# marsermd/DeepestScatter

Measured on AMD Instinct MI355X. Metric: Msamples/s (rays x spp) at 512^3 vol, 1024^2 frame; HBM GB/s vs roofline, higher is better.
Workload: dtype f32

## Files before the change

### deepestscatter_amd/_lib.py

```python
from __future__ import annotations

import ctypes as C
import os
from pathlib import Path

PKG = Path(__file__).resolve().parent
LIB_PATH = PKG / os.path.basename(os.environ.get("CT_LIBRARY", "libcloudtrace.so"))

CT_ABI_VERSION = 1
CT_OK, CT_E_INVAL, CT_E_HIP, CT_E_NOMEM, CT_E_STATE, CT_E_NODEVICE, CT_E_RCCL = 0, -1, -2, -3, -4, -5, -6
CT_MODE_SUN_AND_SKY_ALL_SCATTER, CT_MODE_SUN_MULTIPLE_SCATTER, CT_MODE_SUN_SINGLE_SCATTER = 0, 1, 2
CT_EST_MARCH, CT_EST_DELTA = 0, 1
CT_BUF_MEAN, CT_BUF_M2, CT_BUF_FRAME, CT_BUF_SCREEN, CT_BUF_INSCATTER, CT_BUF_DENSITY = range(6)
CT_FLAG_NONE, CT_FLAG_SIMPLE_KERNEL, CT_FLAG_LIGHT_NORMALIZED, CT_FLAG_SPARSE_BRICKS, CT_FLAG_VMM_BRICKS = 0, 1, 2, 4, 8
CT_FLAG_TEX_FIXED8 = 16

EXPORTS = [
    "ct_create", "ct_destroy", "ct_last_error", "ct_set_stream", "ct_set_camera", "ct_render_subframe",
    "ct_accumulate", "ct_render_accumulate", "ct_render_accumulate_async", "ct_synchronize", "ct_copy_to_device_async", "ct_point_radiance_launch", "ct_generate_scatter_samples", "ct_collect_descriptors", "ct_reset", "ct_tonemap", "ct_tonemap_async", "ct_set_render_ahead", "ct_rendered_subframes", "ct_set_stop_when_converged", "ct_converged_at", "ct_is_converged", "ct_tonemap_buffer", "ct_is_converged_buffers", "ct_download", "ct_upload",
    "ct_buffer_bytes", "ct_copy_to_device", "ct_device_ptr", "ct_subframes", "ct_set_subframes", "ct_counters", "ct_kernel_time",
    "ct_debug_cdf_inversion", "ct_debug_math_selftest", "ct_debug_fetch_probe", "ct_debug_fetch_probe_ws", "ct_debug_track_lines", "ct_debug_touched_lines", "ct_debug_stats", "ct_debug_stats_ex", "ct_debug_suspended", "ct_debug_timeline", "ct_debug_invariants", "ct_debug_memory", "ct_debug_delta_grid", "ct_debug_march_meta", "ct_fetch_counters", "ct_calculate_camera_variables", "ct_quantize_volume", "ct_load_vdb", "ct_generate_mipmaps",
    "ct_tile_owner", "ct_make_procedural_cloud",
    "ct_group_create", "ct_group_destroy", "ct_group_last_error", "ct_group_size", "ct_group_handle", "ct_group_set_camera",
    "ct_group_render_accumulate", "ct_group_reset", "ct_group_merge", "ct_group_download", "ct_group_tonemap",
    "ct_group_is_converged", "ct_group_counters",
]


class CtScene(C.Structure):
    _fields_ = [
        ("abi_version", C.c_uint32),
        ("dims", C.c_uint32 * 3),
        ("density_host", C.c_void_p),
        ("cloud_size_m", C.c_float),
        ("mean_free_path_m", C.c_float),
        ("sample_step", C.c_float),
# ... 86 lines not shown
        "ct_copy_to_device": (i32, [vp, i32, vp, C.c_size_t]),
        "ct_copy_to_device_async": (i32, [vp, i32, vp, C.c_size_t]),
        "ct_debug_suspended": (i32, [vp, vp]),
        "ct_debug_timeline": (i32, [vp, vp, u32]),
        "ct_device_ptr": (i32, [vp, i32, C.POINTER(vp)]),
        "ct_subframes": (i32, [vp, C.POINTER(u32)]),
        "ct_set_subframes": (i32, [vp, u32]),
        "ct_counters": (i32, [vp, C.POINTER(CtCounters)]),
        "ct_kernel_time": (i32, [vp, C.POINTER(C.c_double), C.POINTER(C.c_double), C.POINTER(C.c_uint64)]),
        "ct_debug_cdf_inversion": (i32, [vp, u32, u32, vp]),
        "ct_debug_math_selftest": (i32, [vp, i32, vp]),
        "ct_debug_stats": (i32, [vp, vp]),
        "ct_debug_stats_ex": (i32, [vp, vp, C.c_uint32]),
        "ct_debug_invariants": (i32, [vp, vp]),
        "ct_debug_memory": (i32, [vp, vp]),
        "ct_debug_delta_grid": (i32, [vp, vp]),
        "ct_debug_march_meta": (i32, [vp, vp, vp, C.c_size_t]),
        "ct_fetch_counters": (i32, [vp, C.POINTER(CtFetchCounters)]),
        "ct_debug_fetch_probe": (i32, [i32, u32, u32, C.POINTER(C.c_uint64)]),
        "ct_debug_fetch_probe_ws": (i32, [i32, u32, C.c_uint64, u32, C.POINTER(C.c_uint64)]),
        "ct_debug_track_lines": (i32, [vp, i32]),
        "ct_debug_touched_lines": (i32, [vp, C.POINTER(C.c_uint64), i32]),
        "ct_calculate_camera_variables": (i32, [vp, vp, vp, f32, f32, vp, vp, vp]),
        "ct_quantize_volume": (i32, [vp, vp, vp]),
        "ct_load_vdb": (i32, [C.c_char_p, vp, vp, C.c_size_t, C.POINTER(C.c_size_t), C.c_char_p, C.c_size_t]),
        "ct_generate_mipmaps": (i32, [vp, vp, vp, C.c_size_t, C.POINTER(u32), C.POINTER(C.c_size_t), vp]),
        "ct_tile_owner": (u32, [u32, u32, u32]),
        "ct_group_create": (i32, [C.POINTER(CtScene), vp, u32, C.POINTER(vp)]),
        "ct_group_destroy": (i32, [vp]),
        "ct_group_last_error": (C.c_char_p, [vp]),
# ... 25 lines not shown
```

### deepestscatter_amd/cloudtrace.py

```python
from __future__ import annotations

import ctypes as C
from dataclasses import dataclass
from pathlib import Path

import numpy as np

from . import _lib
from ._lib import (CT_BUF_DENSITY, CT_BUF_FRAME, CT_BUF_INSCATTER, CT_BUF_M2, CT_BUF_MEAN, CT_BUF_SCREEN,
                   CtCounters, CtFetchCounters, CtScene, check)

MIE_FILE = Path(__file__).resolve().parent / "data" / "mie_raw.f32"

LIGHT_DIRECTIONS = {
    "Front": (-0.586, -0.766, -0.271),
    "Side": (-0.03, -0.25, 0.8),
    "Back": (0.586, -0.766, -0.271),
}


def load_mie_raw() -> tuple[np.ndarray, np.ndarray]:
    raw = np.fromfile(MIE_FILE, dtype="<f4")
    if raw.size != 8192:
        raise RuntimeError(f"{MIE_FILE} is corrupt")
# ... 338 lines not shown
        c = CtFetchCounters()
        check(self.L.ct_fetch_counters(self.h, C.byref(c)), self.h)
        return c.as_dict()

    def debug_invariants(self) -> dict:
        out = np.zeros(8, np.uint64)
        check(self.L.ct_debug_invariants(self.h, _p(out)), self.h)
        names = ["armed", "checks", "violations", "samples_without_alpha_1", "dealt", "resumed", "written", "suspended"]
        return {n: int(v) for n, v in zip(names, out)}

    def debug_memory(self) -> dict:
        out = np.zeros(8, np.uint64)
        check(self.L.ct_debug_memory(self.h, _p(out)), self.h)
        names = ["raw_texture", "density_bricks", "inscatter_bricks", "march_bricks_dense", "march_bricks_stored", "sparse",
                 "row_table", "coarse_clearance"]
        return {n: int(v) for n, v in zip(names, out)}

    def delta_grid(self) -> dict:
        out = np.zeros(8, np.uint32)
        check(self.L.ct_debug_delta_grid(self.h, _p(out)), self.h)
        return {"cell": int(out[0]), "stored": tuple(int(v) for v in out[1:4]), "origin": tuple(int(v) for v in out[4:7]),
                "nee": int(out[7] & 0xff), "interior": bool(out[7] & 0x100)}

    def march_meta(self) -> dict:
        geom = np.zeros(8, np.uint32)
        check(self.L.ct_debug_march_meta(self.h, _p(geom), C.c_void_p(), 0), self.h)
        d = {"radius": int(geom[0]), "bias_x": int(geom[1]), "bias": int(geom[2]),
             "bricks": tuple(int(v) for v in geom[3:6]), "sparse": bool(geom[6]), "meta": None}
        if not d["sparse"]:
            gx, gy, gz = d["bricks"]
# ... 8 lines not shown
        return float(a.value), float(b.value), int(n.value)

    def set_stream(self, hip_stream: int | None):
        check(self.L.ct_set_stream(self.h, C.c_void_p(hip_stream) if hip_stream else None), self.h)

    def debug_stats(self) -> dict:
        out = np.zeros(64, np.uint64)
        check(self.L.ct_debug_stats(self.h, _p(out)), self.h)
        names = ["regen_phases", "regen_lanes", "march_phases", "march_lanes", "scatter_phases", "scatter_lanes",
                 "fetched_steps", "fetched_zero_cells", "skipped_steps", "zero_cells_nonfree_brick",
                 "zero_cells_free_brick_d1", "skip_loop_wave_iterations", "nee_footprints_reused", "waves",
                 "stolen_jobs", "max_scheduler_visits_of_a_wave"]
        d = {n: int(v) for n, v in zip(names, out)}
        d["wave_end_hist_5ms"] = [int(v) for v in out[16:40]]
        d["wave_end_minus_drained_hist_0p5ms"] = [int(v) for v in out[40:64]]
        ex = np.zeros(73, np.uint64)
        check(self.L.ct_debug_stats_ex(self.h, _p(ex), 73), self.h)
        d["march_fetch_same_line_as_lanes_previous"] = int(ex[68])
        d["march_fetch_line_shared_with_a_lower_lane"] = int(ex[69])
        d["nee_lookups_skipped_shadow_zero"] = int(ex[72])
        d["raw"] = [int(v) for v in out]
        d["watchdog"] = int(out[63])
        return d

    def debug_suspended(self) -> int:
        n = C.c_uint64(0)
        check(self.L.ct_debug_suspended(self.h, C.byref(n)), self.h)
        return int(n.value)

    def debug_math_selftest(self, which: int) -> dict:
        out = np.zeros(3, np.uint64)
        check(self.L.ct_debug_math_selftest(self.h, which, _p(out)), self.h)
        return {"tested": int(out[0]), "mismatches": int(out[1]), "first_bad_bits": int(out[2])}

    def debug_cdf_inversion(self, first_u24: int, count: int) -> np.ndarray:
# ... 81 lines not shown
```

### deepestscatter_amd/csrc/ct_api.cpp

```cpp
#include <algorithm>
#include <array>
#include <atomic>
#include <chrono>
#include <climits>
#include <cmath>
#include <cstdarg>
#include <cstdio>
#include <cstdlib>
#include <cstring>
#include <new>
#include <string>
#include <utility>
#include <map>
#include <vector>

#include "../../include/cloudtrace.h"
#include "ct_internal.hpp"

using namespace ct;

struct Knob {
    bool is_set = false;
    std::string text;
    const char *get() const { return is_set ? text.c_str() : nullptr; }
    explicit operator bool() const { return is_set; }
};
#define CT_KNOBS(X) X(BURST_IDLE) X(BURST_MARCH_MIN) X(BURST_SCATTER) X(CHUNK_INTERLEAVE) X(CHUNK_MORTON) X(CONTINUATION) X(DEBUG_INVARIANTS) X(DELTA_INTERIOR) X(DELTA_NEE) X(EXCHANGE) X(HAND_ON_JOBS) X(HINT_PERIOD) X(JOB_MAX) X(JOB_WORK) X(MARCH_BURST) X(MAX_AGE) X(NEE_CACHE) X(NO_ADVANCE) X(POINT_BLOCKS_PER_CU) X(POINT_ORDER) X(REGEN_MIN) X(RENDER_AHEAD) X(SCATTER_MIN) X(SCATTER_RATIO) X(SCRATCH_GIB) X(SCRATCH_MIB) X(SERPENTINE) X(SHARED_DEPTH) X(SPARSE) X(STATS) X(TAIL_BURST) X(TILE_ORDER) X(TIMELINE) X(TRACE) X(TUNE_SUBFRAMES) X(XCD_QUEUES) X(XCD_QUEUES_UNTUNED) X(XCD_REGIONS) X(BLOCKS_PER_CU)
struct CtTuning {
#define X(name) Knob name;
    CT_KNOBS(X)
#undef X
    static CtTuning from_env()
    {
        CtTuning t;
#define X(name)                                  \
    if (const char *e = getenv("CT_" #name)) {   \
        t.name.is_set = true;                    \
        t.name.text = e;                         \
    }
        CT_KNOBS(X)
#undef X
        return t;
// ... 70 lines not shown
    uint64_t scratch_cap_bytes = 0;
    uint32_t layout_S = 0;
    uint32_t *left[2] = { nullptr, nullptr };
    size_t left_capacity = 0;
    uint32_t *d_cont_count = nullptr;
    unsigned long long *d_cont_total = nullptr;
    size_t cont_capacity = 0;
    hipEvent_t ev_flush0 = nullptr, ev_flush1 = nullptr;
    bool continuation = true;
    int max_age_override = 0;
    bool hand_on_jobs = true;
    bool serpentine = false;
    float4 *d_primary = nullptr;
    float4 *d_advance = nullptr;
    uint32_t *d_pixels = nullptr;
    uint8_t *d_hit = nullptr, *hit_host = nullptr;
    uint32_t *d_cost = nullptr;
    uint32_t *d_touched[2] = { nullptr, nullptr };
    size_t touched_lines[2] = { 0, 0 };
    unsigned long long *d_timeline = nullptr;
    uint2 *d_cost_plane = nullptr;
    size_t cost_plane_capacity = 0;
    uint32_t *d_job_group = nullptr, *d_job_sub = nullptr;
    uint32_t n_groups = 0, groups_capacity = 0;
    uint32_t n_jobs = 0, jobs_capacity = 0, jobs_S = 0;
    uint32_t *jobs_host_g = nullptr, *jobs_host_s = nullptr;
    size_t jobs_host_capacity = 0;
    bool jobs_brief = false;
    uint32_t chunk_groups = 0, n_chunks = 0;
    std::vector<std::array<uint32_t, kQueues + 2>> chunk_q_begin;
// ... 258 lines not shown
    if (h->stream) {
        hipStreamSynchronize(h->stream);
    }
#ifdef CT_EXPERIMENTS
    if (h->vmm.va) {
        hipMemUnmap(h->vmm.va, h->vmm.size);
        for (auto &hd : h->vmm.handles) {
            hipMemRelease(hd);
        }
        hipMemAddressFree(h->vmm.va, h->vmm.size);
        h->vmm.va = nullptr;
        h->d_mbricks = nullptr;
    }
#endif
    void *ptrs[] = { h->d_density, h->d_inscatter, h->d_dbricks, h->d_ibricks, h->d_mbricks, h->d_tbricks, h->d_touched[0], h->d_touched[1], h->d_mrows, h->d_mcoarse, h->d_pyramid, h->d_mie, h->d_chopped, h->d_cdf,
                     h->d_guide, h->d_dist, h->d_dist_tmp, h->d_majorant, h->d_maj_cells, h->d_maj_codes, h->d_frame, h->d_mean, h->d_m2, h->d_screen, h->d_frames_all, h->cont[0], h->cont[1], h->left[0], h->left[1], h->d_cont_count, h->d_cont_total, h->d_primary, h->d_advance, h->d_pixels, h->d_cost, h->d_group_rank, h->d_group_order, h->d_job_group, h->d_job_sub, h->d_queue,
                     h->d_counters, h->d_colsum, h->d_avg, h->d_freeze, h->d_hit, h->d_cost_plane, h->d_timeline, h->pt.tasks, h->pt.primary, h->pt.frames, h->pt.pixels, h->pt.jg, h->pt.js };
    for (void *p : ptrs) {
        if (p) {
            hipFree(p);
        }
    }
    for (auto &e : h->ev) {
        if (e) {
            hipEventDestroy(e);
        }
    }
    for (auto &sl : h->slots) {
        if (sl.queue) {
            hipFree(sl.queue);
        }
// ... 358 lines not shown
    }
    if (delta) {
        d.delta_nee = (uint32_t)knob_int(t.DELTA_NEE, 0, 2, big ? 2 : 1);
        h->job_work = 48.f;
    }
    h->queues_enabled = knob_flag(t.XCD_QUEUES, big);
    h->regions = (uint32_t)knob_int(t.XCD_REGIONS, 1, 65536, (int)h->regions);
    if (const char *e = t.SHARED_DEPTH.get()) {
        h->shared_depth = (float)atof(e);
    }
    h->job_max = (uint32_t)knob_int(t.JOB_MAX, 1, 4096, (int)h->job_max);
    if (const char *e = t.JOB_WORK.get()) {
        h->job_work = (float)std::max(1.0, atof(e));
    }
    h->no_advance = knob_flag(t.NO_ADVANCE, h->no_advance);
    h->point_order = knob_flag(t.POINT_ORDER, h->point_order);
    h->continuation = knob_flag(t.CONTINUATION, h->continuation) && !h->exchange;
    h->chunk_interleave = knob_flag(t.CHUNK_INTERLEAVE, h->chunk_interleave);
    if (const char *e = t.TILE_ORDER.get()) {
        h->tile_hilbert = strcmp(e, "hilbert") == 0;
    }
    h->chunk_morton = knob_flag(t.CHUNK_MORTON, h->chunk_morton);
    h->serpentine = knob_flag(t.SERPENTINE, h->serpentine);
    h->hand_on_jobs = knob_flag(t.HAND_ON_JOBS, h->hand_on_jobs);
    h->max_age_override = knob_int(t.MAX_AGE, 0, CtHandle_::kMaxRegions - 1, h->max_age_override);
    h->ahead = (uint32_t)knob_int(t.RENDER_AHEAD, 0, 65535, (int)h->ahead);
    return CT_OK;
}

static void scene_uniforms(const CtScene *s, DevScene &d)
// ... 479 lines not shown
    NEED(h);
    if (!eye || !U || !V || !W) {
        return fail(h, CT_E_INVAL, "camera vectors must not be NULL");
    }
    DevScene &d = h->dev;
    d.ex = eye[0]; d.ey = eye[1]; d.ez = eye[2];
    d.ux = U[0]; d.uy = U[1]; d.uz = U[2];
    d.vx = V[0]; d.vy = V[1]; d.vz = V[2];
    d.wx = W[0]; d.wy = W[1]; d.wz = W[2];
    h->camera_set = true;
    h->queue_dirty = true;
    discard_ahead(h);
    return CT_OK;
}

static int rebuild_queue(CtHandle h)
{
    TracePhase trace(h, "rebuild_queue");
    const uint32_t W = h->scene.width, H = h->scene.height;
    const size_t pixels = (size_t)W * H;
    HIPCHK(h, launch_primary_rays(h->dev, h->d_primary, h->stream));
    if (h->scene.estimator == CT_EST_DELTA) {
        HIPCHK(h, launch_primary_advance_delta(h->dev, h->d_primary, h->d_advance, h->stream));
    } else {
        HIPCHK(h, launch_primary_advance(h->dev, h->d_primary, h->d_advance, h->stream));
    }
    if (!h->d_hit) {
        HIPCHK(h, dmalloc(&h->d_hit, pixels));
        HIPCHK(h, hipHostMalloc((void **)&h->hit_host, pixels, hipHostMallocDefault));
    }
// ... 67 lines not shown
                c >>= 1;
            }
            return k;
        };
        std::stable_sort(h->group_order.begin(), h->group_order.end(), [&](uint32_t a, uint32_t b) {
            return log2_class(h->tile_deepest[h->group_tile[a]]) > log2_class(h->tile_deepest[h->group_tile[b]]);
        });
    }
    h->group_depth.assign(h->n_groups, 0.f);
    if (h->n_groups) {
        HIPCHK(h, hipMemcpyAsync(h->d_pixels, list.data(), list.size() * sizeof(uint32_t), hipMemcpyHostToDevice,
                                 h->stream));
        HIPCHK(h, hipMemsetAsync(h->d_cost, 0, 2 * (size_t)h->n_groups * sizeof(uint32_t), h->stream));
        HIPCHK(h, hipStreamSynchronize(h->stream));
    }
    h->queue_dirty = false;
    h->order_tuned = false;
    h->jobs_S = 0;
    return CT_OK;
}

static bool short_batch(CtHandle h, uint32_t S)
{
    return h->scene.estimator != CT_EST_DELTA && (double)S * (double)std::max<uint64_t>(h->hit_pixels, 1) < 4.0e7;
}

static int build_jobs(CtHandle h, uint32_t S, uint32_t chunk_groups)
{
    chunk_groups = std::max(1u, std::min(chunk_groups, std::max(h->n_groups, 1u)));
    if (h->jobs_S >= S && h->jobs_brief == short_batch(h, S) && h->chunk_groups == chunk_groups) {
// ... 439 lines not shown
        } else {
            HIPCHK(h, launch_render_delta_x(sc, ba, h->xshape, h->stream));
        }
        launched = true;
    }
#endif
    if (launched) {
    } else if (h->scene.estimator == CT_EST_DELTA) {
        HIPCHK(h, launch_render_delta(sc, ba, h->shape, h->stream));
    } else {
        HIPCHK(h, launch_render_persistent(sc, ba, h->shape, h->stream));
    }
    return CT_OK;
}

static int submit_batch(CtHandle h, int slot, float4 *dense_frames, uint32_t first, uint32_t S, bool accumulate,
                        bool suspend, uint32_t chunk)
{
    CtHandle_::Slot &sl = h->slots[slot];
    const bool simple = (h->scene.flags & CT_FLAG_SIMPLE_KERNEL) != 0;
    const bool dense = dense_frames != nullptr;
    const uint32_t max_age = (uint32_t)(h->n_regions - 1);
    const uint32_t rank_base = chunk * h->chunk_groups;
    const uint32_t chunk_n = h->n_groups > rank_base ? std::min(h->chunk_groups, h->n_groups - rank_base) : 0u;
    BatchArgs ba{};
    ba.frames = dense ? dense_frames : (simple ? slot_frames(h, slot) : h->d_frames_all);
    ba.frame_stride = (simple || dense) ? 0u : (uint32_t)frame_stride(h);
    ba.out_offset = (simple || dense) ? 0u : (uint32_t)((size_t)slot * h->slot_capacity);
    ba.primary = h->d_primary;
    ba.advance = h->no_advance ? nullptr : h->d_advance;
    ba.pixels = h->d_pixels;
    ba.group_rank = (simple || dense || h->n_chunks <= 1) ? nullptr : h->d_group_rank;
    ba.rank_base = rank_base;
    ba.job_group = h->d_job_group;
    ba.job_sub = h->d_job_sub;
    const bool measure = !h->order_tuned && !simple && !dense && chunk_n != 0u;
    if (measure) {
        const size_t entries = (size_t)S * frame_stride(h);
        if (entries > h->cost_plane_capacity) {
            if (h->d_cost_plane) {
                HIPCHK(h, hipFree(h->d_cost_plane));
                h->d_cost_plane = nullptr;
            }
            h->cost_plane_capacity = entries + entries / 4;
            HIPCHK(h, dmalloc(&h->d_cost_plane, h->cost_plane_capacity));
        }
// ... 139 lines not shown
        return fail(h, CT_E_STATE, "invariant violated: dealt %llu (expected %llu) resumed %llu written %llu suspended %llu bad samples %llu",
                    dealt, (unsigned long long)h->iv_expected_dealt, resumed, written, suspended, bad);
    }
    return CT_OK;
}

static int flush(CtHandle h)
{
    if (h->cont_live) {
        BatchArgs ba{};
        ba.frames = h->d_frames_all;
        ba.frame_stride = (uint32_t)frame_stride(h);
        ba.primary = h->d_primary;
        ba.advance = h->no_advance ? nullptr : h->d_advance;
        ba.pixels = h->d_pixels;
        ba.job_group = h->d_job_group;
        ba.job_sub = h->d_job_sub;
        ba.n_jobs = 0;
        ba.first_subframe = 1;
        ba.S = 0;
        ba.queue = h->d_queue;
        ba.counters = h->d_counters;
        ba.stats = h->d_counters + kCounterCount + 1;
        const int buf_in = (int)((h->launch_no & 1u) ^ 1u);
        ba.cont_in = h->cont[buf_in];
        ba.cont_in_count = h->d_cont_count + buf_in;
        ba.cont_cursor = h->d_cont_count + 2;
        ba.left_in = h->left[buf_in];
        ba.left_in_count = h->d_cont_count + 3 + buf_in;
        ba.left_cursor = h->d_cont_count + 5;
// ... 1004 lines not shown
    if (!out) {
        return fail(h, CT_E_INVAL, "out is NULL");
    }
    const size_t brick_bytes = (size_t)h->dev.brick_gxy * (size_t)h->dev.brick_gz * 128;
    out[0] = h->volume_bytes;
    out[1] = brick_bytes;
    out[2] = brick_bytes;
    out[3] = h->mbricks_dense_bytes;
    out[4] = h->mbricks_bytes;
    out[5] = h->dev.m_rows ? 1 : (h->vmm.va ? 2 : 0);
    out[6] = h->dev.m_rows ? (size_t)h->dev.brick_gy * h->dev.brick_gz * sizeof(uint2) : 0;
    out[7] = h->dev.m_rows ? (size_t)h->dev.m_cgxy * (size_t)((4 * h->dev.brick_gz + 7) >> h->dev.m_cshift) : 0;
    return CT_OK;
}

extern "C" int ct_debug_delta_grid(CtHandle h, uint32_t out[8])
{
    NEED(h);
    if (!out) {
        return fail(h, CT_E_INVAL, "out is NULL");
    }
    const DevScene &d = h->dev;
    const bool delta = d.maj_cells != nullptr;
    out[0] = delta ? (uint32_t)d.mc_cell : 0u;
    out[1] = delta ? (uint32_t)d.mc_gx : 0u;
    out[2] = delta ? (uint32_t)d.mc_gy : 0u;
    out[3] = delta ? (uint32_t)d.mc_gz : 0u;
    out[4] = delta ? (uint32_t)d.mc_x0 : 0u;
    out[5] = delta ? (uint32_t)d.mc_y0 : 0u;
    out[6] = delta ? (uint32_t)d.mc_z0 : 0u;
// ... 181 lines not shown
```

### deepestscatter_amd/csrc/ct_internal.hpp

```cpp
#pragma once

#include <hip/hip_runtime.h>
#include <stdint.h>

#include "ct_device.hpp"

namespace ct {

constexpr int kTile = 8;
constexpr int kCounterCount = 9;
constexpr int kStatCount = 73;
constexpr int kContWords = 16;
constexpr int kContWordsDelta = 32;
constexpr int kLeftWords = 8;
constexpr int kQueueFlag = 32;
constexpr int kQueueDone = 16;
constexpr int kQueueWords = 64;
constexpr int kQueues = 8;

struct BatchArgs {
    float4 *frames;
    uint32_t frame_stride;
    const float4 *primary;
    const float4 *advance;
    const uint32_t *pixels;
    const uint32_t *group_rank;
    uint32_t rank_base;
    const uint32_t *job_group;
    const uint32_t *job_sub;
    uint2 *cost;
    uint32_t n_jobs;
    uint32_t q_begin[kQueues + 2];
    uint32_t reverse;
    uint32_t first_subframe;
    uint32_t S;
    uint32_t *queue;
    const uint32_t *cont_in;
    const uint32_t *cont_in_count;
    uint32_t *cont_cursor;
// ... 57 lines not shown
#endif
hipError_t launch_mbrick_extent(const uint8_t *bricks, int gx, int gy, int gz, uint32_t *row_x0, uint32_t *row_x1, hipStream_t stream);
hipError_t launch_mbrick_compact(const uint8_t *dense, int gx, int gy, int gz, const uint2 *rows, uint8_t *compact, hipStream_t stream);
hipError_t launch_nee_skip_flags(const uint8_t *shadow, int nx, int ny, int nz, int r, int bias_x, int bias, int gx, int gy,
                                 int gz, uint8_t *tmp_a, uint8_t *tmp_c, uint8_t *bricks, hipStream_t stream);
hipError_t launch_coarse_clearance(const uint8_t *dist, int nx, int ny, int nz, int bias, int cshift, int cgx, int cgy, int cgz,
                                   uint8_t *out, hipStream_t stream);
hipError_t launch_render_delta(const DevScene &sc, const BatchArgs &ba, LaunchShape shape, hipStream_t stream);
hipError_t launch_inscatter(const DevScene &sc, uint8_t *out, uint32_t zero_faces, hipStream_t stream);
hipError_t launch_primary_rays(const DevScene &sc, float4 *primary, hipStream_t stream);
hipError_t launch_cost_reduce(const uint2 *cost_plane, uint32_t frame_stride, uint32_t S, uint32_t n_groups_in_chunk,
                              const uint32_t *group_order, uint32_t rank_base, uint32_t *cost_sum, uint32_t *cost_deepest,
                              hipStream_t stream);
hipError_t launch_hit_flags(const float4 *primary, uint8_t *flags, uint32_t pixels, hipStream_t stream);
hipError_t launch_primary_advance(const DevScene &sc, const float4 *primary, float4 *advance, hipStream_t stream);
hipError_t launch_primary_advance_delta(const DevScene &sc, const float4 *primary, float4 *advance, hipStream_t stream);
struct ZeroList {
    uint32_t *ptr[6];
    uint32_t words[6];
    int n = 0;
    void add(uint32_t *p, uint32_t w) { ptr[n] = p; words[n] = w; n += 1; }
};
hipError_t launch_zero_words(const ZeroList &z, hipStream_t stream);
hipError_t launch_fill_frame(float4 *frame, uint32_t width, uint32_t height, uint32_t shard_index,
                             uint32_t shard_count, hipStream_t stream);
hipError_t launch_render_persistent(const DevScene &sc, const BatchArgs &ba, LaunchShape shape, hipStream_t stream);
hipError_t launch_render_simple(const DevScene &sc, const BatchArgs &ba, uint32_t shard_index,
                                uint32_t shard_count, hipStream_t stream);
hipError_t launch_accumulate_batch(const float4 *frames, float4 *mean, float4 *m2, uint32_t first_subframe,
                                   uint32_t S, uint32_t width, uint32_t height, uint32_t shard_index,
// ... 49 lines not shown
```

### deepestscatter_amd/csrc/ct_kernels.hip

```cpp
#include <algorithm>
#include <cstdlib>

#include "ct_internal.hpp"

namespace ct {

__global__ void build_bricks_kernel(const uint8_t *__restrict__ t, int nx, int ny, int nz, int bias,
                                    uint8_t *__restrict__ bricks, int gx, int gy, int gz)
{
    const int64_t total = (int64_t)gx * gy * gz * 128;
    for (int64_t i = (int64_t)blockIdx.x * blockDim.x + threadIdx.x; i < total; i += (int64_t)gridDim.x * blockDim.x) {
        const int64_t b = i >> 7;
        const int o = (int)(i & 127);
        uint8_t v = 0;
        if (o < 125) {
            const int lx = o % 5, ly = (o / 5) % 5, lz = o / 25;
            const int x = (int)(b % gx) * 4 + lx - bias;
            const int y = (int)((b / gx) % gy) * 4 + ly - bias;
            const int z = (int)(b / ((int64_t)gx * gy)) * 4 + lz - bias;
            const int xc = min(max(x, 0), nx - 1), yc = min(max(y, 0), ny - 1), zc = min(max(z, 0), nz - 1);
            v = t[((size_t)zc * ny + yc) * nx + xc];
        }
        bricks[i] = v;
    }
// ... 942 lines not shown
    }
    advance[p] = make_float4(start.x, start.y, start.z, __uint_as_float(start_bits));
}

hipError_t launch_primary_advance(const DevScene &sc, const float4 *primary, float4 *advance, hipStream_t stream)
{
    const dim3 grid((sc.width + 31) / 32, (sc.height + 7) / 8), block(256);
    if (sc.m_rows) {
        hipLaunchKernelGGL(primary_advance_kernel<true>, grid, block, 0, stream, sc, primary, advance);
    } else {
        hipLaunchKernelGGL(primary_advance_kernel<false>, grid, block, 0, stream, sc, primary, advance);
    }
    return hipGetLastError();
}

template <int MODE, bool STATS, bool SPARSE, bool COST = true, bool FIXED8 = false>
__global__ __launch_bounds__(512) __attribute__((amdgpu_waves_per_eu(6))) void render_persistent_kernel(DevScene sc, BatchArgs ba)
{
    __shared__ MieLdsFull lds;
    load_tables(sc, lds);

    const uint32_t lane = threadIdx.x & 63u;
#ifdef CT_DIAG_TIMELINE
    if (ba.timeline && lane == 0u) {
        ba.timeline[4u * (blockIdx.x * (blockDim.x >> 6) + (threadIdx.x >> 6))] = wall_clock64();
    }
#endif
    f3 pos = mk3(0, 0, 0), dir = mk3(0, 0, 1), stepv = mk3(0, 0, 0), rad = mk3(0, 0, 0);
    uint32_t seed = 0, depth = 0, out_idx = 0;
    uint32_t work = 0;
// ... 4 lines not shown

    JobState job{ 0, 0, 0, 0, 0, 0 };
    bool left_done = false;
    uint32_t q_cur = (uint32_t)kQueues, q_tried = 0;
    bool drained = false;
    uint32_t c_dl = 0, c_il = 0, c_cap = 0;
    uint32_t w_fetch = 0, w_nee = 0;
    uint32_t iv_dealt = 0, iv_written = 0, iv_resumed = 0, iv_suspended = 0;
    uint32_t nee_key = 0xffffffffu;
    uint2 nee_cell = make_uint2(0u, 0u);
    uint32_t st_regen = 0, st_regen_l = 0, st_march = 0, st_march_l = 0, st_scat = 0, st_scat_l = 0;
    uint32_t st_fetch = 0, st_zero = 0, st_skip = 0, st_zero_d0 = 0, st_zero_d1 = 0, st_skip_iters = 0, st_stolen = 0, st_iters = 0, st_first = 0;
    uint32_t st_hit2 = 0, st_hit3 = 0, st_h2 = 0xffffffffu, st_h3 = 0xffffffffu;
    uint32_t st_same_line = 0, st_dup_line = 0, st_prev_line = 0xffffffffu;
    uint32_t st_nee_zero = 0;

    uint32_t age = 0;
    if (ba.cont_in) {
        const uint32_t total = __builtin_amdgcn_readfirstlane(*ba.cont_in_count);
        uint32_t base = 0;
        if (lane == 0) {
            base = atomicAdd(ba.cont_cursor, 64u);
        }
        base = __builtin_amdgcn_readfirstlane(base);
        if (base + lane < total) {
            const uint4 *e = (const uint4 *)(ba.cont_in + (size_t)(base + lane) * kContWords);
            const uint4 w0 = e[0], w1 = e[1], w2 = e[2], w3 = e[3];
            pos = mk3(__uint_as_float(w0.x), __uint_as_float(w0.y), __uint_as_float(w0.z));
            dir = mk3(__uint_as_float(w0.w), __uint_as_float(w1.x), __uint_as_float(w1.y));
            rad = mk3(__uint_as_float(w1.z), __uint_as_float(w1.w), __uint_as_float(w2.x));
// ... 107 lines not shown
                        }
                        bool go = hit && in_box(sc, pos);
                        if (MODE != 2 && go) {
                            depth = 1;
                            if (depth == sc.max_depth) {
                                c_cap += 1;
                                go = false;
                            }
                        }
                        if (go) {
                            xi = u24_to_float(lcg24(seed));
                            T = 1;
                            stepv = scale3(dir, sc.sample_step);
                            inv_maxd = inv_max_advance(sc, stepv);
                            dfree = 0;
                            if (MODE != 1 && ba.advance) {
                                const float4 a = ba.advance[pixel];
                                const uint32_t bits = __float_as_uint(a.w);
                                pos = mk3(a.x, a.y, a.z);
                                dfree = bits >> 24;
                                c_dl += bits & 0x00ffffffu;
                            }
                            state = ST_MARCH;
                        } else {
                            ba.frames[out_idx] = make_float4(0.f, 0.f, 0.f, 1.f);
                            if (STATS) {
                                iv_written += 1;
                            }
                        }
                    }
                }
            }
        }

        const uint64_t marching = __builtin_amdgcn_ballot_w64(state == ST_MARCH);
        const uint64_t bouncing = __builtin_amdgcn_ballot_w64(state == ST_BOUNCE);
        const uint32_t nm = (uint32_t)__builtin_popcountll(marching);
        const uint32_t nb = (uint32_t)__builtin_popcountll(bouncing);
// ... 88 lines not shown
        if (track) {
            if (STATS) {
                st_march += 1;
                st_march_l += nm_track;
            }
            w_fetch += nm_track;
            uint32_t burst = drained ? sc.tail_burst : sc.march_burst;
            for (;;) {
            if (state == ST_MARCH) {
                if (dfree != 0u) {
                    const int n = skip_steps(dfree, inv_maxd);
                    replay_steps(pos, stepv, n);
                    c_dl += (uint32_t)n;
                    if (STATS) {
                        st_skip += (uint32_t)n;
                        int wmax = n;
#pragma unroll
                        for (int off = 32; off > 0; off >>= 1) {
                            wmax = max(wmax, __shfl_xor(wmax, off));
                        }
                        st_skip_iters += (lane_rank(__builtin_amdgcn_ballot_w64(true)) == 0u) ? (uint32_t)wmax : 0u;
                    }
                }
                pos = add3(pos, stepv);
                uint32_t meta;
                const uint2 cell = fetch_cell_m<SPARSE>(sc, pos, meta);
                dfree = meta & 0x3fu;
                c_dl += 1;
                if (COST) {
                    work += 1u;
                }
                if (STATS) {
                    st_fetch += 1;
                    {
                        const float fx = fmaf(pos.x, sc.sx, -0.5f), fy = fmaf(pos.y, sc.sy, -0.5f), fz = fmaf(pos.z, sc.sz, -0.5f);
                        const uint32_t lx = (uint32_t)(floor_to_int(fx) + sc.m_bias_x), ly = (uint32_t)(floor_to_int(fy) + sc.brick_bias),
                                       lz = (uint32_t)(floor_to_int(fz) + sc.brick_bias);
                        const uint32_t line = __umul24(lz >> 2, (uint32_t)sc.m_gxy) + __umul24(ly >> 2, (uint32_t)sc.m_gx) + (__umul24(lx, 43691u) >> 17);
                        st_same_line += (line == st_prev_line) ? 1u : 0u;
                        st_prev_line = line;
                        if (ba.touched_density && !SPARSE) {
                            atomicOr(&ba.touched_density[line >> 5], 1u << (line & 31u));
                        }
                        const uint64_t act = __builtin_amdgcn_ballot_w64(true);
                        bool dup = false;
                        for (uint32_t i = 0; i < 64u; i++) {
                            const uint32_t other = (uint32_t)__builtin_amdgcn_readlane((int)line, (int)i);
                            dup = dup || (((act >> i) & 1ull) != 0ull && i < lane && other == line);
// ... 89 lines not shown
                    if (STATS) {
                        iv_suspended += 1;
                    }
                }
            }
        }
    }

#ifdef CT_DIAG_TIMELINE
    if (ba.timeline && lane == 0u) {
        ba.timeline[4u * (blockIdx.x * (blockDim.x >> 6) + (threadIdx.x >> 6)) + 1u] = wall_clock64();
    }
#endif
    const uint32_t vals[3] = { wave_sum(c_dl), wave_sum(c_il), wave_sum(c_cap) };
    if (STATS) {
        uint32_t sv[16] = { st_fetch, st_zero, st_skip, st_zero_d0, st_zero_d1, st_skip_iters, st_first,
                            iv_dealt, iv_resumed, iv_written, iv_suspended, st_same_line, st_dup_line, st_hit2, st_hit3, st_nee_zero };
#pragma unroll
        for (int i = 0; i < 16; i++) {
            sv[i] = wave_sum(sv[i]);
        }
        if (lane == 0) {
            atomicAdd(&ba.stats[0], (unsigned long long)st_regen);
            atomicAdd(&ba.stats[1], (unsigned long long)st_regen_l);
            atomicAdd(&ba.stats[2], (unsigned long long)st_march);
            atomicAdd(&ba.stats[3], (unsigned long long)st_march_l);
            atomicAdd(&ba.stats[4], (unsigned long long)st_scat);
            atomicAdd(&ba.stats[5], (unsigned long long)st_scat_l);
            atomicAdd(&ba.stats[6], (unsigned long long)sv[0]);
            atomicAdd(&ba.stats[7], (unsigned long long)sv[1]);
            atomicAdd(&ba.stats[8], (unsigned long long)sv[2]);
            atomicAdd(&ba.stats[9], (unsigned long long)sv[3]);
            atomicAdd(&ba.stats[10], (unsigned long long)sv[4]);
            atomicAdd(&ba.stats[11], (unsigned long long)sv[5]);
// ... 6 lines not shown
            atomicAdd(&ba.stats[16 + min((unsigned long long)23, (t_end - t_start) / 25000ull)], 1ull);
            atomicAdd(&ba.stats[40 + min((unsigned long long)23, (t_end - (t_drained ? t_drained : t_end)) / 5000ull)], 1ull);
#else
            atomicAdd(&ba.stats[16 + min((unsigned long long)23, (t_end - t_start) / 500000ull)], 1ull);
            atomicAdd(&ba.stats[40 + min((unsigned long long)23, (t_end - (t_drained ? t_drained : t_end)) / 50000ull)], 1ull);
#endif
            atomicAdd(&ba.stats[64], (unsigned long long)sv[7]);
            atomicAdd(&ba.stats[65], (unsigned long long)sv[8]);
            atomicAdd(&ba.stats[66], (unsigned long long)sv[9]);
            atomicAdd(&ba.stats[67], (unsigned long long)sv[10]);
            atomicAdd(&ba.stats[68], (unsigned long long)sv[11]);
            atomicAdd(&ba.stats[69], (unsigned long long)sv[12]);
            atomicAdd(&ba.stats[70], (unsigned long long)sv[13]);
            atomicAdd(&ba.stats[71], (unsigned long long)sv[14]);
            atomicAdd(&ba.stats[72], (unsigned long long)sv[15]);
        }
    }
    flush_counters(ba, lane, vals[0], vals[1], vals[2], w_fetch, w_nee);
}

__global__ void mip_level_kernel(const uint8_t *__restrict__ prev, int px, int py, int pz, uint8_t *__restrict__ cur,
                                 int cx, int cy, int cz)
{
    const int64_t total = (int64_t)cx * cy * cz;
    for (int64_t i = (int64_t)blockIdx.x * blockDim.x + threadIdx.x; i < total; i += (int64_t)gridDim.x * blockDim.x) {
        const int x = (int)(i % cx), y = (int)((i / cx) % cy), z = (int)(i / ((int64_t)cx * cy));
        uint32_t acc = 0;
#pragma unroll
        for (int d = 0; d < 8; d++) {
            const int sx = 2 * x + (d & 1), sy = 2 * y + ((d >> 1) & 1), sz = 2 * z + (d >> 2);
// ... 1547 lines not shown
```

### include/cloudtrace.h

```cpp
#ifndef CLOUDTRACE_H
#define CLOUDTRACE_H

#include <stddef.h>
#include <stdint.h>

#ifdef __cplusplus
extern "C" {
#endif

#define CT_ABI_VERSION 1

#if defined(__GNUC__)
#define CT_API __attribute__((visibility("default")))
#else
#define CT_API
#endif

typedef enum CtStatus {
    CT_OK = 0,
    CT_E_INVAL = -1,
    CT_E_HIP = -2,
    CT_E_NOMEM = -3,
    CT_E_STATE = -4,
    CT_E_NODEVICE = -5,
// ... 155 lines not shown
CT_API int ct_counters(CtHandle h, CtCounters *out);

CT_API int ct_fetch_counters(CtHandle h, CtFetchCounters *out);

CT_API int ct_kernel_time(CtHandle h, double *render_ms_out, double *accumulate_ms_out, uint64_t *launches_out);

CT_API int ct_debug_stats(CtHandle h, uint64_t out[64]);
CT_API int ct_debug_stats_ex(CtHandle h, uint64_t *out, uint32_t count);
CT_API int ct_debug_timeline(CtHandle h, uint64_t *out, uint32_t waves);

CT_API int ct_debug_suspended(CtHandle h, uint64_t *paths_out);

CT_API int ct_debug_invariants(CtHandle h, uint64_t out[8]);

CT_API int ct_debug_memory(CtHandle h, uint64_t out[8]);

CT_API int ct_debug_delta_grid(CtHandle h, uint32_t out[8]);

CT_API int ct_debug_march_meta(CtHandle h, uint32_t geom_out[8], uint8_t *meta_out, size_t capacity);

CT_API int ct_debug_fetch_probe(int32_t device, uint32_t log2_lines, uint32_t repeats, uint64_t *sum_out);

CT_API int ct_debug_fetch_probe_ws(int32_t device, uint32_t log2_threads, uint64_t ws_lines, uint32_t repeats, uint64_t *sum_out);

CT_API int ct_debug_track_lines(CtHandle h, int32_t enable);
CT_API int ct_debug_touched_lines(CtHandle h, uint64_t out[4], int32_t clear);

CT_API int ct_debug_math_selftest(CtHandle h, int32_t which, uint64_t out[3]);

CT_API int ct_debug_cdf_inversion(CtHandle h, uint32_t first_u24, uint32_t count, uint32_t *k_host_out);
// ... 39 lines not shown
```

Before: 3677.

## Precompute per-pixel primary march transmittance table and invert it per sample

Adds a precomputed table that, for each primary pixel, records up to a fixed number of march steps with their transmittance, step bits, position and density. At path start the render kernel inverts the random number against this table with a vectorised compare instead of re-marching the first flight through the volume. This is meant to remove repeated density fetches on the deterministic first segment, which is identical across samples per pixel. In exchange it costs extra device memory, a build kernel on every queue rebuild, and extra table reads per path. It is enabled by default, except with the delta estimator or when advance is disabled.

```diff
diff --git a/deepestscatter_amd/_lib.py b/deepestscatter_amd/_lib.py
--- a/deepestscatter_amd/_lib.py
+++ b/deepestscatter_amd/_lib.py
@@ -19,7 +19,7 @@
     "ct_create", "ct_destroy", "ct_last_error", "ct_set_stream", "ct_set_camera", "ct_render_subframe",
     "ct_accumulate", "ct_render_accumulate", "ct_render_accumulate_async", "ct_synchronize", "ct_copy_to_device_async", "ct_point_radiance_launch", "ct_generate_scatter_samples", "ct_collect_descriptors", "ct_reset", "ct_tonemap", "ct_tonemap_async", "ct_set_render_ahead", "ct_rendered_subframes", "ct_set_stop_when_converged", "ct_converged_at", "ct_is_converged", "ct_tonemap_buffer", "ct_is_converged_buffers", "ct_download", "ct_upload",
     "ct_buffer_bytes", "ct_copy_to_device", "ct_device_ptr", "ct_subframes", "ct_set_subframes", "ct_counters", "ct_kernel_time",
-    "ct_debug_cdf_inversion", "ct_debug_math_selftest", "ct_debug_fetch_probe", "ct_debug_fetch_probe_ws", "ct_debug_track_lines", "ct_debug_touched_lines", "ct_debug_stats", "ct_debug_stats_ex", "ct_debug_suspended", "ct_debug_timeline", "ct_debug_invariants", "ct_debug_memory", "ct_debug_delta_grid", "ct_debug_march_meta", "ct_fetch_counters", "ct_calculate_camera_variables", "ct_quantize_volume", "ct_load_vdb", "ct_generate_mipmaps",
+    "ct_debug_cdf_inversion", "ct_debug_math_selftest", "ct_debug_fetch_probe", "ct_debug_fetch_probe_ws", "ct_debug_track_lines", "ct_debug_touched_lines", "ct_debug_stats", "ct_debug_stats_ex", "ct_debug_suspended", "ct_debug_timeline", "ct_debug_invariants", "ct_debug_memory", "ct_debug_primary_table", "ct_debug_delta_grid", "ct_debug_march_meta", "ct_fetch_counters", "ct_calculate_camera_variables", "ct_quantize_volume", "ct_load_vdb", "ct_generate_mipmaps",
     "ct_tile_owner", "ct_make_procedural_cloud",
     "ct_group_create", "ct_group_destroy", "ct_group_last_error", "ct_group_size", "ct_group_handle", "ct_group_set_camera",
     "ct_group_render_accumulate", "ct_group_reset", "ct_group_merge", "ct_group_download", "ct_group_tonemap",
@@ -136,6 +136,7 @@
         "ct_debug_stats_ex": (i32, [vp, vp, C.c_uint32]),
         "ct_debug_invariants": (i32, [vp, vp]),
         "ct_debug_memory": (i32, [vp, vp]),
+        "ct_debug_primary_table": (i32, [vp, vp]),
         "ct_debug_delta_grid": (i32, [vp, vp]),
         "ct_debug_march_meta": (i32, [vp, vp, vp, C.c_size_t]),
         "ct_fetch_counters": (i32, [vp, C.POINTER(CtFetchCounters)]),
diff --git a/deepestscatter_amd/cloudtrace.py b/deepestscatter_amd/cloudtrace.py
--- a/deepestscatter_amd/cloudtrace.py
+++ b/deepestscatter_amd/cloudtrace.py
@@ -376,6 +376,14 @@
         check(self.L.ct_debug_memory(self.h, _p(out)), self.h)
         names = ["raw_texture", "density_bricks", "inscatter_bricks", "march_bricks_dense", "march_bricks_stored", "sparse",
                  "row_table", "coarse_clearance"]
+        d = {n: int(v) for n, v in zip(names, out)}
+        d["primary_table"] = self.debug_primary_table()["bytes"]
+        return d
+
+    def debug_primary_table(self) -> dict:
+        out = np.zeros(6, np.uint64)
+        check(self.L.ct_debug_primary_table(self.h, _p(out)), self.h)
+        names = ["bytes", "entries", "slots_per_entry", "recorded_steps", "tables_ending_at_the_box_exit", "tables_cut_short"]
         return {n: int(v) for n, v in zip(names, out)}
 
     def delta_grid(self) -> dict:
@@ -414,11 +422,13 @@
         d = {n: int(v) for n, v in zip(names, out)}
         d["wave_end_hist_5ms"] = [int(v) for v in out[16:40]]
         d["wave_end_minus_drained_hist_0p5ms"] = [int(v) for v in out[40:64]]
-        ex = np.zeros(73, np.uint64)
-        check(self.L.ct_debug_stats_ex(self.h, _p(ex), 73), self.h)
+        ex = np.zeros(75, np.uint64)
+        check(self.L.ct_debug_stats_ex(self.h, _p(ex), 75), self.h)
         d["march_fetch_same_line_as_lanes_previous"] = int(ex[68])
         d["march_fetch_line_shared_with_a_lower_lane"] = int(ex[69])
         d["nee_lookups_skipped_shadow_zero"] = int(ex[72])
+        d["first_flight_fetched_steps"] = int(ex[73])
+        d["first_flight_skipped_steps"] = int(ex[74])
         d["raw"] = [int(v) for v in out]
         d["watchdog"] = int(out[63])
         return d
diff --git a/deepestscatter_amd/csrc/ct_api.cpp b/deepestscatter_amd/csrc/ct_api.cpp
--- a/deepestscatter_amd/csrc/ct_api.cpp
+++ b/deepestscatter_amd/csrc/ct_api.cpp
@@ -25,7 +25,7 @@
     const char *get() const { return is_set ? text.c_str() : nullptr; }
     explicit operator bool() const { return is_set; }
 };
-#define CT_KNOBS(X) X(BURST_IDLE) X(BURST_MARCH_MIN) X(BURST_SCATTER) X(CHUNK_INTERLEAVE) X(CHUNK_MORTON) X(CONTINUATION) X(DEBUG_INVARIANTS) X(DELTA_INTERIOR) X(DELTA_NEE) X(EXCHANGE) X(HAND_ON_JOBS) X(HINT_PERIOD) X(JOB_MAX) X(JOB_WORK) X(MARCH_BURST) X(MAX_AGE) X(NEE_CACHE) X(NO_ADVANCE) X(POINT_BLOCKS_PER_CU) X(POINT_ORDER) X(REGEN_MIN) X(RENDER_AHEAD) X(SCATTER_MIN) X(SCATTER_RATIO) X(SCRATCH_GIB) X(SCRATCH_MIB) X(SERPENTINE) X(SHARED_DEPTH) X(SPARSE) X(STATS) X(TAIL_BURST) X(TILE_ORDER) X(TIMELINE) X(TRACE) X(TUNE_SUBFRAMES) X(XCD_QUEUES) X(XCD_QUEUES_UNTUNED) X(XCD_REGIONS) X(BLOCKS_PER_CU)
+#define CT_KNOBS(X) X(BURST_IDLE) X(BURST_MARCH_MIN) X(BURST_SCATTER) X(CHUNK_INTERLEAVE) X(CHUNK_MORTON) X(CONTINUATION) X(DEBUG_INVARIANTS) X(DELTA_INTERIOR) X(DELTA_NEE) X(EXCHANGE) X(HAND_ON_JOBS) X(HINT_PERIOD) X(JOB_MAX) X(JOB_WORK) X(MARCH_BURST) X(MAX_AGE) X(NEE_CACHE) X(NO_ADVANCE) X(POINT_BLOCKS_PER_CU) X(POINT_ORDER) X(PRIMARY_TABLE) X(PRIMARY_TABLE_CAP) X(REGEN_MIN) X(RENDER_AHEAD) X(SCATTER_MIN) X(SCATTER_RATIO) X(SCRATCH_GIB) X(SCRATCH_MIB) X(SERPENTINE) X(SHARED_DEPTH) X(SPARSE) X(STATS) X(TAIL_BURST) X(TILE_ORDER) X(TIMELINE) X(TRACE) X(TUNE_SUBFRAMES) X(XCD_QUEUES) X(XCD_QUEUES_UNTUNED) X(XCD_REGIONS) X(BLOCKS_PER_CU)
 struct CtTuning {
 #define X(name) Knob name;
     CT_KNOBS(X)
@@ -126,6 +126,11 @@
     float4 *d_primary = nullptr;
     float4 *d_advance = nullptr;
     uint32_t *d_pixels = nullptr;
+    uint32_t *d_ptab = nullptr;
+    size_t ptab_words = 0;
+    uint32_t ptab_entries = 0;
+    uint32_t ptab_cap = 32;
+    bool primary_table = true;
     uint8_t *d_hit = nullptr, *hit_host = nullptr;
     uint32_t *d_cost = nullptr;
     uint32_t *d_touched[2] = { nullptr, nullptr };
@@ -414,7 +419,7 @@
     }
 #endif
     void *ptrs[] = { h->d_density, h->d_inscatter, h->d_dbricks, h->d_ibricks, h->d_mbricks, h->d_tbricks, h->d_touched[0], h->d_touched[1], h->d_mrows, h->d_mcoarse, h->d_pyramid, h->d_mie, h->d_chopped, h->d_cdf,
-                     h->d_guide, h->d_dist, h->d_dist_tmp, h->d_majorant, h->d_maj_cells, h->d_maj_codes, h->d_frame, h->d_mean, h->d_m2, h->d_screen, h->d_frames_all, h->cont[0], h->cont[1], h->left[0], h->left[1], h->d_cont_count, h->d_cont_total, h->d_primary, h->d_advance, h->d_pixels, h->d_cost, h->d_group_rank, h->d_group_order, h->d_job_group, h->d_job_sub, h->d_queue,
+                     h->d_guide, h->d_dist, h->d_dist_tmp, h->d_majorant, h->d_maj_cells, h->d_maj_codes, h->d_frame, h->d_mean, h->d_m2, h->d_screen, h->d_frames_all, h->cont[0], h->cont[1], h->left[0], h->left[1], h->d_cont_count, h->d_cont_total, h->d_primary, h->d_advance, h->d_pixels, h->d_ptab, h->d_cost, h->d_group_rank, h->d_group_order, h->d_job_group, h->d_job_sub, h->d_queue,
                      h->d_counters, h->d_colsum, h->d_avg, h->d_freeze, h->d_hit, h->d_cost_plane, h->d_timeline, h->pt.tasks, h->pt.primary, h->pt.frames, h->pt.pixels, h->pt.jg, h->pt.js };
     for (void *p : ptrs) {
         if (p) {
@@ -803,6 +808,8 @@
         h->job_work = (float)std::max(1.0, atof(e));
     }
     h->no_advance = knob_flag(t.NO_ADVANCE, h->no_advance);
+    h->primary_table = knob_flag(t.PRIMARY_TABLE, h->primary_table) && !h->no_advance && !delta;
+    h->ptab_cap = (uint32_t)knob_int(t.PRIMARY_TABLE_CAP, 1, 64, (int)h->ptab_cap);
     h->point_order = knob_flag(t.POINT_ORDER, h->point_order);
     h->continuation = knob_flag(t.CONTINUATION, h->continuation) && !h->exchange;
     h->chunk_interleave = knob_flag(t.CHUNK_INTERLEAVE, h->chunk_interleave);
@@ -1312,6 +1319,37 @@
     return CT_OK;
 }
 
+static uint32_t ptab_stride(CtHandle h) { return (h->ptab_cap + 7u) & ~7u; }
+
+static int build_primary_table(CtHandle h)
+{
+    h->ptab_entries = 0;
+    if (!h->primary_table || h->scene.estimator == CT_EST_DELTA || (h->scene.flags & CT_FLAG_SIMPLE_KERNEL) || h->n_groups == 0) {
+        return CT_OK;
+    }
+    const uint32_t entries = h->n_groups * 64u;
+    const size_t words = (size_t)entries * (1 + 6 * (size_t)ptab_stride(h));
+    if (words >= ((size_t)1 << 32)) {
+        return CT_OK;
+    }
+    if (words > h->ptab_words) {
+        if (h->d_ptab) {
+            HIPCHK(h, hipFree(h->d_ptab));
+            h->d_ptab = nullptr;
+            h->ptab_words = 0;
+        }
+        if (dmalloc(&h->d_ptab, words) != hipSuccess) {
+            (void)hipGetLastError();
+            h->d_ptab = nullptr;
+            return CT_OK;
+        }
+        h->ptab_words = words;
+    }
+    HIPCHK(h, launch_primary_table(h->dev, h->d_primary, h->d_advance, h->d_pixels, entries, h->ptab_cap, ptab_stride(h), h->d_ptab, h->stream));
+    h->ptab_entries = entries;
+    return CT_OK;
+}
+
 static int rebuild_queue(CtHandle h)
 {
     TracePhase trace(h, "rebuild_queue");
@@ -1409,6 +1447,7 @@
         HIPCHK(h, hipMemsetAsync(h->d_cost, 0, 2 * (size_t)h->n_groups * sizeof(uint32_t), h->stream));
         HIPCHK(h, hipStreamSynchronize(h->stream));
     }
+    CT_TRY(build_primary_table(h));
     h->queue_dirty = false;
     h->order_tuned = false;
     h->jobs_S = 0;
@@ -1878,6 +1917,13 @@
     return CT_OK;
 }
 
+static void set_primary_table(CtHandle h, BatchArgs &ba)
+{
+    ba.ptab = h->ptab_entries ? h->d_ptab : nullptr;
+    ba.ptab_stride = ptab_stride(h);
+    ba.ptab_entries = h->ptab_entries;
+}
+
 static int submit_batch(CtHandle h, int slot, float4 *dense_frames, uint32_t first, uint32_t S, bool accumulate,
                         bool suspend, uint32_t chunk)
 {
@@ -1894,6 +1940,7 @@
     ba.primary = h->d_primary;
     ba.advance = h->no_advance ? nullptr : h->d_advance;
     ba.pixels = h->d_pixels;
+    set_primary_table(h, ba);
     ba.group_rank = (simple || dense || h->n_chunks <= 1) ? nullptr : h->d_group_rank;
     ba.rank_base = rank_base;
     ba.job_group = h->d_job_group;
@@ -2063,6 +2110,7 @@
         ba.primary = h->d_primary;
         ba.advance = h->no_advance ? nullptr : h->d_advance;
         ba.pixels = h->d_pixels;
+        set_primary_table(h, ba);
         ba.job_group = h->d_job_group;
         ba.job_sub = h->d_job_sub;
         ba.n_jobs = 0;
@@ -3097,6 +3145,30 @@
     return CT_OK;
 }
 
+extern "C" int ct_debug_primary_table(CtHandle h, uint64_t out[6])
+{
+    NEED(h);
+    if (!out) {
+        return fail(h, CT_E_INVAL, "out is NULL");
+    }
+    out[0] = h->ptab_words * sizeof(uint32_t);
+    out[1] = h->ptab_entries;
+    out[2] = ptab_stride(h);
+    out[3] = out[4] = out[5] = 0;
+    if (h->ptab_entries) {
+        std::vector<uint32_t> head(h->ptab_entries);
+        HIPCHK(h, hipStreamSynchronize(h->stream));
+        HIPCHK(h, hipMemcpy(head.data(), h->d_ptab, head.size() * sizeof(uint32_t), hipMemcpyDeviceToHost));
+        for (uint32_t v : head) {
+            const uint32_t n = v & 0x7fffffffu;
+            out[3] += n;
+            out[4] += (v >> 31) ? 1u : 0u;
+            out[5] += (n != 0u && (v >> 31) == 0u) ? 1u : 0u;
+        }
+    }
+    return CT_OK;
+}
+
 extern "C" int ct_debug_delta_grid(CtHandle h, uint32_t out[8])
 {
     NEED(h);
diff --git a/deepestscatter_amd/csrc/ct_internal.hpp b/deepestscatter_amd/csrc/ct_internal.hpp
--- a/deepestscatter_amd/csrc/ct_internal.hpp
+++ b/deepestscatter_amd/csrc/ct_internal.hpp
@@ -9,7 +9,7 @@
 
 constexpr int kTile = 8;
 constexpr int kCounterCount = 9;
-constexpr int kStatCount = 73;
+constexpr int kStatCount = 75;
 constexpr int kContWords = 16;
 constexpr int kContWordsDelta = 32;
 constexpr int kLeftWords = 8;
@@ -23,6 +23,9 @@
     uint32_t frame_stride;
     const float4 *primary;
     const float4 *advance;
+    const uint32_t *ptab;
+    uint32_t ptab_stride;
+    uint32_t ptab_entries;
     const uint32_t *pixels;
     const uint32_t *group_rank;
     uint32_t rank_base;
@@ -110,6 +113,8 @@
                               hipStream_t stream);
 hipError_t launch_hit_flags(const float4 *primary, uint8_t *flags, uint32_t pixels, hipStream_t stream);
 hipError_t launch_primary_advance(const DevScene &sc, const float4 *primary, float4 *advance, hipStream_t stream);
+hipError_t launch_primary_table(const DevScene &sc, const float4 *primary, const float4 *advance, const uint32_t *pixels,
+                                uint32_t entries, uint32_t cap, uint32_t stride, uint32_t *tab, hipStream_t stream);
 hipError_t launch_primary_advance_delta(const DevScene &sc, const float4 *primary, float4 *advance, hipStream_t stream);
 struct ZeroList {
     uint32_t *ptr[6];
diff --git a/deepestscatter_amd/csrc/ct_kernels.hip b/deepestscatter_amd/csrc/ct_kernels.hip
--- a/deepestscatter_amd/csrc/ct_kernels.hip
+++ b/deepestscatter_amd/csrc/ct_kernels.hip
@@ -980,6 +980,90 @@
     return hipGetLastError();
 }
 
+template <bool SPARSE, bool FIXED8>
+__global__ __launch_bounds__(256) void primary_table_kernel(DevScene sc, const float4 *__restrict__ primary,
+                                                            const float4 *__restrict__ advance,
+                                                            const uint32_t *__restrict__ pixels, uint32_t entries, uint32_t cap,
+                                                            uint32_t stride, uint32_t *__restrict__ tab)
+{
+    const uint32_t e = blockIdx.x * 256u + threadIdx.x;
+    if (e >= entries) {
+        return;
+    }
+    const size_t slots = (size_t)entries * stride;
+    float *t_out = (float *)(tab + entries) + (size_t)e * stride;
+    uint32_t *bits_out = tab + entries + slots + (size_t)e * stride;
+    float4 *pay_out = (float4 *)(tab + entries + 2 * slots) + (size_t)e * stride;
+    uint32_t n = 0, left = 0;
+    const uint32_t pixel = pixels[e];
+    if (pixel != 0xffffffffu) {
+        const float4 p0 = primary[2 * (size_t)pixel], p1 = primary[2 * (size_t)pixel + 1];
+        if (p0.w != 0.f && in_box(sc, mk3(p0.x, p0.y, p0.z))) {
+            const f3 stepv = scale3(mk3(p1.x, p1.y, p1.z), sc.sample_step);
+            const float inv_maxd = inv_max_advance(sc, stepv);
+            const float4 a = advance[pixel];
+            f3 pos = mk3(a.x, a.y, a.z);
+            uint32_t dfree = __float_as_uint(a.w) >> 24, steps = __float_as_uint(a.w) & 0x00ffffffu;
+            float T = 1;
+            while (n < cap && steps < 0x00f00000u) {
+                if (dfree != 0u) {
+                    const int skipped = skip_steps(dfree, inv_maxd);
+                    replay_steps(pos, stepv, skipped);
+                    steps += (uint32_t)skipped;
+                }
+                pos = add3(pos, stepv);
+                steps += 1u;
+                uint32_t meta;
+                const uint2 cell = fetch_cell_m<SPARSE>(sc, pos, meta);
+                dfree = meta & 0x3fu;
+                const float density = filter_at<FIXED8>(sc, cell, pos) * sc.density_multiplier;
+                const float extinction = density * sc.sample_step;
+                const float t_next = T * expf_inrange(-extinction);
+                if (!(t_next <= T)) {
+                    break;
+                }
+                T = t_next;
+                t_out[n] = T;
+                bits_out[n] = steps | ((meta & 0xffu) << 24);
+                pay_out[n] = make_float4(pos.x, pos.y, pos.z, density);
+                n += 1u;
+                if ((meta & 0x80u) == 0u && !in_box(sc, pos)) {
+                    left = 1u;
+                    break;
+                }
+                if (T == 0.f) {
+                    break;
+                }
+            }
+        }
+    }
+    for (uint32_t k = n; k < stride; k++) {
+        t_out[k] = -1.f;
+    }
+    tab[e] = n | (left << 31);
+}
+
+hipError_t launch_primary_table(const DevScene &sc, const float4 *primary, const float4 *advance, const uint32_t *pixels,
+                                uint32_t entries, uint32_t cap, uint32_t stride, uint32_t *tab, hipStream_t stream)
+{
+    const dim3 grid((entries + 255u) / 256u), block(256);
+    if (entries == 0u) {
+        return hipSuccess;
+    }
+    if (sc.m_rows) {
+        if (sc.tex_fixed8) {
+            hipLaunchKernelGGL((primary_table_kernel<true, true>), grid, block, 0, stream, sc, primary, advance, pixels, entries, cap, stride, tab);
+        } else {
+            hipLaunchKernelGGL((primary_table_kernel<true, false>), grid, block, 0, stream, sc, primary, advance, pixels, entries, cap, stride, tab);
+        }
+    } else if (sc.tex_fixed8) {
+        hipLaunchKernelGGL((primary_table_kernel<false, true>), grid, block, 0, stream, sc, primary, advance, pixels, entries, cap, stride, tab);
+    } else {
+        hipLaunchKernelGGL((primary_table_kernel<false, false>), grid, block, 0, stream, sc, primary, advance, pixels, entries, cap, stride, tab);
+    }
+    return hipGetLastError();
+}
+
 template <int MODE, bool STATS, bool SPARSE, bool COST = true, bool FIXED8 = false>
 __global__ __launch_bounds__(512) __attribute__((amdgpu_waves_per_eu(6))) void render_persistent_kernel(DevScene sc, BatchArgs ba)
 {
@@ -1014,6 +1098,7 @@
     uint32_t st_hit2 = 0, st_hit3 = 0, st_h2 = 0xffffffffu, st_h3 = 0xffffffffu;
     uint32_t st_same_line = 0, st_dup_line = 0, st_prev_line = 0xffffffffu;
     uint32_t st_nee_zero = 0;
+    uint32_t st_ff_fetch = 0, st_ff_skip = 0;
 
     uint32_t age = 0;
     if (ba.cont_in) {
@@ -1151,14 +1236,58 @@
                             stepv = scale3(dir, sc.sample_step);
                             inv_maxd = inv_max_advance(sc, stepv);
                             dfree = 0;
-                            if (MODE != 1 && ba.advance) {
+                            state = ST_MARCH;
+                            const uint32_t entry = g * 64u + l;
+                            const uint32_t head = (MODE != 1 && ba.ptab) ? ba.ptab[entry] : 0u;
+                            const uint32_t tab_n = head & 0x7fffffffu;
+                            if (MODE != 1 && tab_n != 0u) {
+                                const uint32_t row = entry * ba.ptab_stride;
+                                const uint32_t *tt = ba.ptab + (ba.ptab_entries + row);
+                                uint32_t k = 0;
+                                for (uint32_t c = 0; c < ba.ptab_stride; c += 8u) {
+                                    float4 ta, tb;
+                                    __builtin_memcpy(&ta, tt + c, sizeof ta);
+                                    __builtin_memcpy(&tb, tt + c + 4u, sizeof tb);
+                                    k += (xi > ta.x ? 0u : 1u) + (xi > ta.y ? 0u : 1u) + (xi > ta.z ? 0u : 1u) + (xi > ta.w ? 0u : 1u) +
+                                         (xi > tb.x ? 0u : 1u) + (xi > tb.y ? 0u : 1u) + (xi > tb.z ? 0u : 1u) + (xi > tb.w ? 0u : 1u);
+                                    if (k < c + 8u) {
+                                        break;
+                                    }
+                                }
+                                const uint32_t at = min(k, tab_n - 1u);
+                                const uint32_t slots = ba.ptab_entries * ba.ptab_stride;
+                                const uint32_t bits = tt[slots + at];
+                                float4 pay;
+                                __builtin_memcpy(&pay, ba.ptab + (ba.ptab_entries + 2u * slots + 4u * (row + at)), sizeof pay);
+                                T = __uint_as_float(tt[at]);
+                                pos = mk3(pay.x, pay.y, pay.z);
+                                c_dl += bits & 0x00ffffffu;
+                                if (COST) {
+                                    work += at + 1u;
+                                }
+                                if (k < tab_n) {
+                                    inv_maxd = pay.w;
+                                    dfree = (bits >> 24) & 0xc0u;
+                                    state = ST_BOUNCE;
+                                } else if ((head >> 31) != 0u) {
+                                    ba.frames[out_idx] = make_float4(0.f, 0.f, 0.f, 1.f);
+                                    if (STATS) {
+                                        iv_written += 1;
+                                    }
+                                    if (COST && ba.cost) {
+                                        ba.cost[out_idx - ba.out_offset] = make_uint2(work, depth);
+                                    }
+                                    state = ST_IDLE;
+                                } else {
+                                    dfree = (bits >> 24) & 0x3fu;
+                                }
+                            } else if (MODE != 1 && ba.advance) {
                                 const float4 a = ba.advance[pixel];
                                 const uint32_t bits = __float_as_uint(a.w);
                                 pos = mk3(a.x, a.y, a.z);
                                 dfree = bits >> 24;
                                 c_dl += bits & 0x00ffffffu;
                             }
-                            state = ST_MARCH;
                         } else {
                             ba.frames[out_idx] = make_float4(0.f, 0.f, 0.f, 1.f);
                             if (STATS) {
@@ -1277,6 +1406,7 @@
                     c_dl += (uint32_t)n;
                     if (STATS) {
                         st_skip += (uint32_t)n;
+                        st_ff_skip += (MODE == 2 || depth == 1u) ? (uint32_t)n : 0u;
                         int wmax = n;
 #pragma unroll
                         for (int off = 32; off > 0; off >>= 1) {
@@ -1295,6 +1425,7 @@
                 }
                 if (STATS) {
                     st_fetch += 1;
+                    st_ff_fetch += (MODE == 2 || depth == 1u) ? 1u : 0u;
                     {
                         const float fx = fmaf(pos.x, sc.sx, -0.5f), fy = fmaf(pos.y, sc.sy, -0.5f), fz = fmaf(pos.z, sc.sz, -0.5f);
                         const uint32_t lx = (uint32_t)(floor_to_int(fx) + sc.m_bias_x), ly = (uint32_t)(floor_to_int(fy) + sc.brick_bias),
@@ -1414,10 +1545,11 @@
 #endif
     const uint32_t vals[3] = { wave_sum(c_dl), wave_sum(c_il), wave_sum(c_cap) };
     if (STATS) {
-        uint32_t sv[16] = { st_fetch, st_zero, st_skip, st_zero_d0, st_zero_d1, st_skip_iters, st_first,
-                            iv_dealt, iv_resumed, iv_written, iv_suspended, st_same_line, st_dup_line, st_hit2, st_hit3, st_nee_zero };
+        uint32_t sv[18] = { st_fetch, st_zero, st_skip, st_zero_d0, st_zero_d1, st_skip_iters, st_first,
+                            iv_dealt, iv_resumed, iv_written, iv_suspended, st_same_line, st_dup_line, st_hit2, st_hit3, st_nee_zero,
+                            st_ff_fetch, st_ff_skip };
 #pragma unroll
-        for (int i = 0; i < 16; i++) {
+        for (int i = 0; i < 18; i++) {
             sv[i] = wave_sum(sv[i]);
         }
         if (lane == 0) {
@@ -1454,6 +1586,8 @@
             atomicAdd(&ba.stats[70], (unsigned long long)sv[13]);
             atomicAdd(&ba.stats[71], (unsigned long long)sv[14]);
             atomicAdd(&ba.stats[72], (unsigned long long)sv[15]);
+            atomicAdd(&ba.stats[73], (unsigned long long)sv[16]);
+            atomicAdd(&ba.stats[74], (unsigned long long)sv[17]);
         }
     }
     flush_counters(ba, lane, vals[0], vals[1], vals[2], w_fetch, w_nee);
diff --git a/include/cloudtrace.h b/include/cloudtrace.h
--- a/include/cloudtrace.h
+++ b/include/cloudtrace.h
@@ -193,6 +193,7 @@
 CT_API int ct_debug_invariants(CtHandle h, uint64_t out[8]);
 
 CT_API int ct_debug_memory(CtHandle h, uint64_t out[8]);
+CT_API int ct_debug_primary_table(CtHandle h, uint64_t out[6]);
 
 CT_API int ct_debug_delta_grid(CtHandle h, uint32_t out[8]);
 
```

After: 3686, median of 6. Within noise of the previous version (+0.2%).
